# yuriyvnv/speech_transcript_embeddings

Measured on AMD Instinct MI355X. Metric: audio–text pairs/sec (whole node), 10s@16kHz + 64-tok, 1/2/4/8 MI355X, higher is better.
Workload: dtype bf16; 1 GPU; c2: global batch 64 = 1 GPU x 1 micro-batch(es) of 64 pairs, each pair 10s@16kHz audio + 64-tok clean + 64-tok corrupt; w2v-bert-2.0 Conformer 24L + XLM-R-base 12L, 3+3 unfrozen; GPU fbank -> fwd -> InfoNCE -> bwd -> allreduce -> clip+AdamW; global_batch=64, local_batch=64, micro_batch=64, accumulation_steps=1, seq_len_audio_frames=499, seq_len_text=64, parallelism=dp1

## Files before the change

speech_transcript_embeddings_amd/csrc/gemm.hip:

```cpp
#include <atomic>
#include <cstdio>
#include <utility>
#include "common.h"
#include "../../include/ste.h"

namespace {


STE_DEV int km_chunk_xor(int k) { return ((k & 3) | ((k >> 1) & 4)) << 1; }

STE_DEV float apply_act(float v, int act) {
  switch (act) {
    case STE_ACT_SWISH: return swish_f(v);
    case STE_ACT_GELU: return gelu_f(v);
    case STE_ACT_TANH: return tanhf(v);
    case STE_ACT_RELU: return fmaxf(v, 0.0f);
    default: return v;
  }
}
STE_DEV float act_grad(float z, int act) {
  switch (act) {
    case STE_ACT_SWISH_BWD: return swish_d(z);
    case STE_ACT_GELU_BWD: return gelu_d(z);
    case STE_ACT_TANH_BWD_OUT: return 1.0f - z * z;
// ... 449 lines not shown
template <int EF, int ACT, bool FULL>
STE_DEV void epilogue_bf16s(const ste_gemm_args& p, const f32x4 (&acc)[8][4], char* slot, int m0, int n0, int batch,
                            int wm, int wn, int lane_in, const f32x4 (&bias)[4]) {
  static_assert(epi_bf16s<EF>(), "single bf16 output, no operand loads");
  int lane = lane_in;
  asm volatile("" : "+v"(lane));
  constexpr bool FWD = ACT >= STE_ACT_SWISH && ACT <= STE_ACT_RELU;
  const int64_t offC = (int64_t)batch * p.strideC;
  const int c0 = n0 + wn * 32, c1 = n0 + 128 + wn * 32;
  const int rbase = m0 + wm * 128;
  const float alpha = p.alpha;
#pragma unroll
  for (int ps = 0; ps < 4; ++ps) {
    auto value = [&](int ii, int j) {
      f32x4 x = acc[2 * ps + ii][j];
      if constexpr ((EF & EF_BIAS) != 0) x += bias[j];
      x *= alpha;
      if (FWD) x = act4(x, ACT);
      return x;
    };
    bf16s_pass<FULL>(slot, value, (bf16*)p.C + offC, p.ldc, rbase + 2 * ps * 16, p.M, p.N, c0, c1, lane);
  }
}

#ifndef STE_TILE_GROUP
#define STE_TILE_GROUP 8
#endif
STE_HD void tile_of(int t, int num_m, int num_n, int& tm, int& tn) {
  constexpr int GROUP = STE_TILE_GROUP;
  const int group = t / (GROUP * num_n);
  const int first_m = group * GROUP;
  const int gsize = num_m - first_m < GROUP ? num_m - first_m : GROUP;
  tm = first_m + (t % (GROUP * num_n)) % gsize;
  tn = (t % (GROUP * num_n)) / gsize;
}
STE_DEV void map_tile_bid(int bid, int num_m, int num_n, int& batch, int& tm, int& tn) {
  const int tiles = num_m * num_n;
  batch = bid / tiles;
  tile_of(bid - batch * tiles, num_m, num_n, tm, tn);
}
STE_DEV void map_tile(int nwg, int num_m, int num_n, int& batch, int& tm, int& tn) {
  map_tile_bid(xcd_remap(blockIdx.x, nwg), num_m, num_n, batch, tm, tn);
}

namespace small {
constexpr int BM = 128, BN = 128, BK = 64, NT = 256;
constexpr int TILE_BYTES = BM * BK * 2;
constexpr int EPI_BYTES = 4 * 64 * EPI_LD * 4;
constexpr int LDS_BYTES = (4 * TILE_BYTES > EPI_BYTES) ? 4 * TILE_BYTES : EPI_BYTES;

struct Stage {
  bf16x8 v[4];
};

template <bool KC>
STE_DEV void stage_load(Stage& st, const bf16* __restrict__ base, int64_t ld, int row0, int rows, int k0, int K,
                        int tid) {
#pragma unroll
  for (int i = 0; i < 4; ++i) {
    int c = tid + NT * i;
    int r, kk;
    bool ok;
    const bf16* p;
    if (KC) {
      r = c >> 3; kk = (c & 7) * 8;
      ok = (row0 + r < rows) && (k0 + kk < K);
      p = base + (int64_t)(row0 + r) * ld + (k0 + kk);
    } else {
      kk = c >> 4; r = (c & 15) * 8;
      ok = (k0 + kk < K) && (row0 + r < rows);
      p = base + (int64_t)(k0 + kk) * ld + (row0 + r);
    }
    if (ok) st.v[i] = *reinterpret_cast<const bf16x8*>(p);
    else st.v[i] = bf16x8{};
  }
}

template <bool KC>
STE_DEV void stage_store(const Stage& st, char* tile, int tid) {
#pragma unroll
  for (int i = 0; i < 4; ++i) {
    int c = tid + NT * i;
    int off;
    if (KC) {
      int r = c >> 3, ch = c & 7;
      off = r * 128 + ((ch ^ (r & 7)) << 4);
    } else {
      int k = c >> 4, ch = c & 15;
      off = k * 256 + ((ch ^ km_chunk_xor(k)) << 4);
    }
    *reinterpret_cast<bf16x8*>(tile + off) = st.v[i];
  }
}
}

template <bool KC, int KM_ROW_BYTES>
STE_DEV bf16x8 frag_load(const char* tile, int rb, int s, int lane) {
  if (KC) {
    int r = rb + (lane & 15);
    int ch = s * 4 + (lane >> 4);
    return *reinterpret_cast<const bf16x8*>(tile + r * 128 + ((ch ^ (r & 7)) << 4));
  } else {
    int g = lane >> 4, li = lane & 15, q = li >> 2, p = li & 3;
    int k = s * 32 + 8 * g + q;
    int quad = (rb >> 2) + p;
    int a0 = k * KM_ROW_BYTES + ((quad ^ (km_chunk_xor(k) << 1)) << 3);
    int k1 = k + 4;
    int a1 = k1 * KM_ROW_BYTES + ((quad ^ (km_chunk_xor(k1) << 1)) << 3);
    s16x4 lo = ds_read_tr16(tile + a0);
    s16x4 hi = ds_read_tr16(tile + a1);
    return join_tr(lo, hi);
  }
}

template <bool A_KC, bool B_KC>
__global__ __launch_bounds__(small::NT, 2) void gemm_bf16_kernel(ste_gemm_args p) {
  using namespace small;
  extern __shared__ __attribute__((aligned(16))) char smem[];
  const int tid = threadIdx.x, lane = tid & 63, wave = tid >> 6;
  const int wm = wave >> 1, wn = wave & 1;
  const int num_m = (p.M + BM - 1) / BM, num_n = (p.N + BN - 1) / BN;
  int batch, tm, tn;
  map_tile(gridDim.x, num_m, num_n, batch, tm, tn);
  const int m0 = tm * BM, n0 = tn * BN;
  const bf16* A = (const bf16*)p.A + (int64_t)batch * p.strideA;
  const bf16* B = (const bf16*)p.B + (int64_t)batch * p.strideB;

  f32x4 acc[4][4];
#pragma unroll
  for (int i = 0; i < 4; ++i)
#pragma unroll
    for (int j = 0; j < 4; ++j) acc[i][j] = f32x4{0.f, 0.f, 0.f, 0.f};

  const int nk = (p.K + BK - 1) / BK;
  Stage sa, sb;
  stage_load<A_KC>(sa, A, p.lda, m0, p.M, 0, p.K, tid);
  stage_load<B_KC>(sb, B, p.ldb, n0, p.N, 0, p.K, tid);
  stage_store<A_KC>(sa, smem, tid);
  stage_store<B_KC>(sb, smem + TILE_BYTES, tid);
  __syncthreads();

  for (int kt = 0; kt < nk; ++kt) {
    const int cur = kt & 1;
    const bool more = kt + 1 < nk;
    if (more) {
      stage_load<A_KC>(sa, A, p.lda, m0, p.M, (kt + 1) * BK, p.K, tid);
      stage_load<B_KC>(sb, B, p.ldb, n0, p.N, (kt + 1) * BK, p.K, tid);
    }
    const char* ta = smem + cur * 2 * TILE_BYTES;
    const char* tb = ta + TILE_BYTES;
#pragma unroll
    for (int s = 0; s < 2; ++s) {
      bf16x8 fa[4], fb[4];
#pragma unroll
      for (int i = 0; i < 4; ++i) fa[i] = frag_load<A_KC, 256>(ta, wm * 64 + i * 16, s, lane);
#pragma unroll
      for (int j = 0; j < 4; ++j) fb[j] = frag_load<B_KC, 256>(tb, wn * 64 + j * 16, s, lane);
#pragma unroll
      for (int i = 0; i < 4; ++i)
#pragma unroll
        for (int j = 0; j < 4; ++j) acc[i][j] = mfma16(fa[i], fb[j], acc[i][j]);
    }
    if (more) {
      char* na = smem + (cur ^ 1) * 2 * TILE_BYTES;
      stage_store<A_KC>(sa, na, tid);
      stage_store<B_KC>(sb, na + TILE_BYTES, tid);
    }
    __syncthreads();
  }

  float* epi = reinterpret_cast<float*>(smem) + wave * 64 * EPI_LD;
#pragma unroll
  for (int i = 0; i < 4; ++i)
#pragma unroll
    for (int j = 0; j < 4; ++j)
#pragma unroll
      for (int r = 0; r < 4; ++r)
        epi[(i * 16 + (lane >> 4) * 4 + r) * EPI_LD + j * 16 + (lane & 15)] = acc[i][j][r];
  __builtin_amdgcn_s_waitcnt(0xc07f);
  __builtin_amdgcn_wave_barrier();
  Csum csum = {};
  epilogue_tile(p, epi, 64, m0 + wm * 64, n0 + wn * 64, n0 + wn * 64 + 32, batch, lane, csum);
  if (p.colsum)
    colsum_flush(p, csum, n0 + wn * 64, n0 + wn * 64 + 32, batch, lane, ((int64_t)batch * num_m + tm) * 2 + wm);
}

namespace ph8 {
constexpr int NT = 512;
constexpr int HALF = 16384;
constexpr int BUF = 4 * HALF;
constexpr int RING_BYTES = 2 * BUF;
constexpr int EPI_OFF = RING_BYTES;
constexpr int LDS_BYTES = EPI_OFF + 8 * 16 * 64 * 4;

template <int G>
STE_DEV int half_row(int pr, int h) {
  if (G == 128) return h * 128 + pr;
  return (pr / G) * (2 * G) + h * G + (pr % G);
}

template <bool KC, int G, bool O32 = false>
STE_DEV void stage_half(const bf16* base, int64_t ld, int row0, int rows, int k0, int h, char* dst, int wave,
                        int lane) {
#pragma unroll
  for (int i = 0; i < 2; ++i) {
    const int piece = wave * 2 + i;
    const bf16* src;
    if (KC) {
      const int pr = piece * 8 + (lane >> 3);
      const int ch = (lane & 7) ^ (lane >> 3);
      const int gr = min(row0 + half_row<G>(pr, h), rows - 1);
      if (O32) src = (const bf16*)((const char*)base + (uint32_t)(((uint32_t)gr * (uint32_t)ld + k0 + ch * 8) * 2u));
      else src = base + (int64_t)gr * ld + k0 + ch * 8;
    } else {
      const int kk = piece * 4 + (lane >> 4);
      const int lc = (lane & 15) ^ km_chunk_xor(kk);
      const int gc = min(row0 + half_row<G>(lc * 8, h), rows - 8);
      src = base + (int64_t)(k0 + kk) * ld + gc;
    }
    __builtin_amdgcn_global_load_lds((const void*)src, (lds_void*)(dst + piece * 1024), 16, 0, 0);
  }
}
constexpr int SC_OFF = EPI_OFF;
constexpr int SC_STAGE = 2048;
STE_DEV void stage_scales(const Mx8Args& mx, int m0, int M, int n0, int N, int t, char* smem, int wave, int lane) {
  const bool isb = wave >= 4;
  const int r = (wave & 3) * 64 + lane;
  const uint8_t* src = isb ? mx.sb + (uint32_t)(min(n0 + r, N - 1) * (uint32_t)mx.lsb + 4 * t)
                           : mx.sa + (uint32_t)(min(m0 + r, M - 1) * (uint32_t)mx.lsa + 4 * t);
  char* dst = smem + SC_OFF + (t & 1) * SC_STAGE + (isb ? 1024 : 0) + (wave & 3) * 256;
  __builtin_amdgcn_global_load_lds((const void*)src, (lds_void*)dst, 4, 0, 0);
}
template <int OFF>
STE_DEV void ds_u8_lo(int& r, uint32_t addr) {
  asm volatile("ds_read_u8_d16 %0, %1 offset:%2" : "+v"(r) : "v"(addr), "i"(OFF) : "memory");
}
template <int OFF>
STE_DEV void ds_u8_hi(int& r, uint32_t addr) {
  asm volatile("ds_read_u8_d16_hi %0, %1 offset:%2" : "+v"(r) : "v"(addr), "i"(OFF) : "memory");
}
template <int OFF>
STE_DEV void ds_u8(int& r, uint32_t addr) {
  asm volatile("ds_read_u8 %0, %1 offset:%2" : "=v"(r) : "v"(addr), "i"(OFF) : "memory");
}
typedef int i32x8 __attribute__((ext_vector_type(8)));
typedef int i32x4m __attribute__((ext_vector_type(4)));
STE_DEV i32x8 frag_mx(const char* tile, int rb, int lane) {
  const int r = rb + (lane & 15), g = lane >> 4;
  const i32x4m lo = *reinterpret_cast<const i32x4m*>(tile + r * 128 + ((g ^ (r & 7)) << 4));
  const i32x4m hi = *reinterpret_cast<const i32x4m*>(tile + r * 128 + (((g + 4) ^ (r & 7)) << 4));
  return i32x8{lo[0], lo[1], lo[2], lo[3], hi[0], hi[1], hi[2], hi[3]};
}
template <typename F, int... I>
STE_DEV void static_for_impl(F& f, std::integer_sequence<int, I...>) {
  (f(std::integral_constant<int, I>{}), ...);
}
template <int N, typename F>
STE_DEV void static_for(F&& f) {
  static_for_impl(f, std::make_integer_sequence<int, N>{});
}
template <int X, int Y>
STE_DEV f32x4 mfma_mx(const i32x8& x, const i32x8& y, f32x4 c, int sx, int sy) {
  return __builtin_amdgcn_mfma_scale_f32_16x16x128_f8f6f4(x, y, c, 0, 0, 0, sx, 0, sy);
}
}

#define STE_BARRIER() asm volatile("s_barrier" ::: "memory")
#ifdef STE_PRIO_STATIC
#define STE_PRIO_HI()
#define STE_PRIO_LO()
#else
#define STE_PRIO_HI() __builtin_amdgcn_s_setprio(1)
#define STE_PRIO_LO() __builtin_amdgcn_s_setprio(0)
#endif
#define STE_VMCNT(n) asm volatile("s_waitcnt vmcnt(" #n ")" ::: "memory")

STE_DEV bf16x8 frag_load_km_asm(const char* tile, int rb, int s, int lane) {
  const int g = lane >> 4, li = lane & 15, q = li >> 2, pp = li & 3;
  const int k = s * 32 + 8 * g + q;
  const int quad = (rb >> 2) + pp;
  const int k1 = k + 4;
  const s16x4 lo = ds_read_tr16_asm(tile + k * 256 + ((quad ^ (km_chunk_xor(k) << 1)) << 3));
  const s16x4 hi = ds_read_tr16_asm(tile + k1 * 256 + ((quad ^ (km_chunk_xor(k1) << 1)) << 3));
  return join_tr(lo, hi);
}
template <bool B_KC>
STE_DEV bf16x8 frag_b_8ph(const char* tile, int rb, int s, int lane) {
  if (B_KC) return frag_load<true, 256>(tile, rb, s, lane);
  return frag_load_km_asm(tile, rb, s, lane);
}
template <bool A_KC>
STE_DEV bf16x8 frag_a_8ph(const char* tile, int rb, int s, int lane) {
  if (A_KC) return frag_load<true, 256>(tile, rb, s, lane);
  return frag_load_km_asm(tile, rb, s, lane);
}
#define STE_LDS_SYNC(ASM)                               \
  do {                                                  \
    if (ASM) {                                          \
      asm volatile("s_waitcnt lgkmcnt(0)" ::: "memory"); \
      __builtin_amdgcn_sched_barrier(0);                \
    }                                                   \
  } while (0)

STE_DEV f32x8 tile_bias(const ste_gemm_args& p, int n0, int wn, int lane) {
  const int cl = (lane & 7) * 8;
  const int col = cl < 32 ? n0 + wn * 32 + cl : n0 + 128 + wn * 32 + (cl - 32);
  const int nval = p.N - col;
  return nval > 0 ? ld8(p.bias + col, false, nval >= 8, nval) : f32x8{};
}

template <int EF, int ACT, bool FULL>
STE_DEV void epilogue_8ph(const ste_gemm_args& p, const f32x4 (&acc)[8][4], float* epi, int m0, int n0, int batch,
                          int wm, int wn, int lane, f32x8 bias, const Q8Out* q8 = nullptr) {
  Csum csum = {};
  const int c0 = n0 + wn * 32, c1 = n0 + 128 + wn * 32;
#define STE_EPI_STAGE(PS)                                                                       \
  {                                                                                             \
    _Pragma("unroll") for (int j = 0; j < 4; ++j) {                                             \
      _Pragma("unroll") for (int r = 0; r < 4; ++r) {                                           \
        const int row = (lane >> 4) * 4 + r, chunk = (4 * j + ((lane & 15) >> 2)) ^ ((r >> 1) & 1); \
        epi[row * 64 + chunk * 4 + (lane & 3)] = acc[PS][j][r];                                 \
      }                                                                                         \
    }                                                                                           \
    __builtin_amdgcn_s_waitcnt(0xc07f);                                                         \
    __builtin_amdgcn_wave_barrier();                                                            \
  }
#define STE_EPI_ROW0(PS) (m0 + wm * 128 + (PS) * 16)
#define STE_EPI_LOAD(PS, L) epi_load16<EF, ACT, FULL>(p, STE_EPI_ROW0(PS), c0, c1, batch, lane, L);
#define STE_EPI_STORE(PS, L)                                                                    \
  epi_store16<EF, ACT, FULL>(p, epi, STE_EPI_ROW0(PS), c0, c1, batch, lane, bias, L, csum, q8); \
  __builtin_amdgcn_s_waitcnt(0xc07f);                                                           \
  __builtin_amdgcn_wave_barrier();
  if constexpr (EF < 0) {
#define STE_EPI_G(PS)                                                                           \
    STE_EPI_STAGE(PS)                                                                           \
    epilogue_tile(p, epi, 16, STE_EPI_ROW0(PS), c0, c1, batch, lane, csum, 64, true, q8);       \
    __builtin_amdgcn_s_waitcnt(0xc07f);                                                         \
    __builtin_amdgcn_wave_barrier();
    STE_EPI_G(0) STE_EPI_G(1) STE_EPI_G(2) STE_EPI_G(3) STE_EPI_G(4) STE_EPI_G(5) STE_EPI_G(6) STE_EPI_G(7)
#undef STE_EPI_G
  } else {
    EpiLoads L0, L1;
    STE_EPI_LOAD(0, L0)
    STE_EPI_STAGE(0) STE_EPI_LOAD(1, L1) STE_EPI_STORE(0, L0)
    STE_EPI_STAGE(1) STE_EPI_LOAD(2, L0) STE_EPI_STORE(1, L1)
    STE_EPI_STAGE(2) STE_EPI_LOAD(3, L1) STE_EPI_STORE(2, L0)
    STE_EPI_STAGE(3) STE_EPI_LOAD(4, L0) STE_EPI_STORE(3, L1)
    STE_EPI_STAGE(4) STE_EPI_LOAD(5, L1) STE_EPI_STORE(4, L0)
    STE_EPI_STAGE(5) STE_EPI_LOAD(6, L0) STE_EPI_STORE(5, L1)
    STE_EPI_STAGE(6) STE_EPI_LOAD(7, L1) STE_EPI_STORE(6, L0)
    STE_EPI_STAGE(7) STE_EPI_STORE(7, L1)
  }
#undef STE_EPI_STAGE
#undef STE_EPI_ROW0
#undef STE_EPI_LOAD
#undef STE_EPI_STORE
  if (EF < 0 ? p.colsum != nullptr : (EF & EF_COLSUM) != 0)
    colsum_flush(p, csum, c0, c1, batch, lane, ((int64_t)batch * ((p.M + 255) >> 8) + (m0 >> 8)) * 2 + wm);
}

#ifndef STE_EPI_PRE
#define STE_EPI_PRE 1
#endif
template <int EF, int ACT, class Pro>
STE_DEV void epilogue_8ph_pre(const ste_gemm_args& p, const f32x4 (&acc)[8][4], float* epi, int m0, int n0, int batch,
                              int wm, int wn, int lane, f32x8 bias, Pro&& prologue) {
  static_assert(EF >= 0 && (EF & (EF_COLSUM | EF_BETA | EF_RS | EF_Q8)) == 0, "EPI_PRE epilogues");
  Csum csum = {};
  const int c0 = n0 + wn * 32, c1 = n0 + 128 + wn * 32;
#define STE_EPI_STAGE(PS)                                                                       \
  {                                                                                             \
    _Pragma("unroll") for (int j = 0; j < 4; ++j) {                                             \
      _Pragma("unroll") for (int r = 0; r < 4; ++r) {                                           \
        const int row = (lane >> 4) * 4 + r, chunk = (4 * j + ((lane & 15) >> 2)) ^ ((r >> 1) & 1); \
        epi[row * 64 + chunk * 4 + (lane & 3)] = acc[PS][j][r];                                 \
      }                                                                                         \
    }                                                                                           \
    __builtin_amdgcn_s_waitcnt(0xc07f);                                                         \
    __builtin_amdgcn_wave_barrier();                                                            \
  }
#define STE_EPI_ROW0(PS) (m0 + wm * 128 + (PS) * 16)
#define STE_EPI_LOAD(PS, L) epi_load16<EF, ACT, true>(p, STE_EPI_ROW0(PS), c0, c1, batch, lane, L);
#define STE_EPI_STORE(PS, L)                                                                    \
  epi_store16<EF, ACT, true>(p, epi, STE_EPI_ROW0(PS), c0, c1, batch, lane, bias, L, csum);     \
  __builtin_amdgcn_s_waitcnt(0xc07f);                                                           \
  __builtin_amdgcn_wave_barrier();
  EpiLoads L0, L1;
  STE_EPI_LOAD(0, L0) STE_EPI_LOAD(1, L1)
  prologue();
  STE_EPI_STAGE(0) STE_EPI_STORE(0, L0) STE_EPI_LOAD(2, L0)
  STE_EPI_STAGE(1) STE_EPI_STORE(1, L1) STE_EPI_LOAD(3, L1)
  STE_EPI_STAGE(2) STE_EPI_STORE(2, L0) STE_EPI_LOAD(4, L0)
  STE_EPI_STAGE(3) STE_EPI_STORE(3, L1) STE_EPI_LOAD(5, L1)
  STE_EPI_STAGE(4) STE_EPI_STORE(4, L0) STE_EPI_LOAD(6, L0)
  STE_EPI_STAGE(5) STE_EPI_STORE(5, L1) STE_EPI_LOAD(7, L1)
  STE_EPI_STAGE(6) STE_EPI_STORE(6, L0)
  STE_EPI_STAGE(7) STE_EPI_STORE(7, L1)
#undef STE_EPI_STAGE
#undef STE_EPI_ROW0
#undef STE_EPI_LOAD
#undef STE_EPI_STORE
}

template <int W, int E>
STE_DEV void vm_wait8(int extra) {
  constexpr int WE = W + E < 63 ? W + E : 63;
  if (E > 0 && extra) asm volatile("s_waitcnt vmcnt(%0)" ::"n"(WE) : "memory");
  else asm volatile("s_waitcnt vmcnt(%0)" ::"n"(W) : "memory");
}

template <bool A_KC, bool B_KC>
STE_DEV void operand_bases(const ste_gemm_args& p, int batch, const bf16*& A, const bf16*& B, int& nk) {
  if (p.ws_bytes < 0) {
    const int kc = p.K / 64, rem = (int)(-p.ws_bytes - 1);
    const int64_t k0 = ((int64_t)batch * kc + (batch < rem ? batch : rem)) * 64;
    A = (const bf16*)p.A + k0 * (A_KC ? 1 : p.lda);
    B = (const bf16*)p.B + k0 * (B_KC ? 1 : p.ldb);
    nk = kc + (batch < rem ? 1 : 0);
    return;
  }
  A = (const bf16*)p.A + (int64_t)batch * p.strideA;
  B = (const bf16*)p.B + (int64_t)batch * p.strideB;
  nk = p.K / 64;
}

template <bool A_KC, bool B_KC, int EF, int ACT, bool MX = false>
__global__ __launch_bounds__(ph8::NT, 1) void gemm_8ph_kernel(ste_gemm_args p, Mx8Args mx) {
  using namespace ph8;
  constexpr int E_ST = epi_stores<EF>();
  constexpr bool SW = epi_bf16s<EF>();
  constexpr int VW = MX ? 9 : 8;
  static_assert(!MX || (A_KC && B_KC), "MX operands are k-contiguous");
  static_assert(VW <= 63, "vmcnt immediate");
  extern __shared__ __attribute__((aligned(16))) char smem[];
  const int tid = threadIdx.x, lane = tid & 63;
  const int wave = __builtin_amdgcn_readfirstlane(tid >> 6);
  const int wm = wave >> 2, wn = wave & 3;
  const int num_m = (p.M + 255) / 256, num_n = (p.N + 255) / 256;
  const int total = num_m * num_n * p.batch;
  int nk = p.K / 64;
  int vb = blockIdx.x;
  if (vb >= total) return;
  int batch, tm, tn;
  map_tile_bid(xcd_remap(vb, total), num_m, num_n, batch, tm, tn);
  int m0 = tm * 256, n0 = tn * 256;
  const bf16* A;
  const bf16* B;
  operand_bases<A_KC, B_KC>(p, batch, A, B, nk);
#define STAGE_A(t, h) \
  stage_half<A_KC, 64, MX>(A, p.lda, m0, p.M, (t) * 64, h, smem + ((t) & 1) * BUF + (h) * HALF, wave, lane)
#define STAGE_B(t, h) \
  stage_half<B_KC, 128, MX>(B, p.ldb, n0, p.N, (t) * 64, h, smem + ((t) & 1) * BUF + (2 + (h)) * HALF, wave, lane)
#define STAGE_S(t) \
  if constexpr (MX) stage_scales(mx, m0, p.M, n0, p.N, (t), smem, wave, lane)
#define STAGE_PROLOGUE()                                                    \
  {                                                                         \
    STAGE_A(0, 0); STAGE_S(0); STAGE_B(0, 0); STAGE_B(0, 1); STAGE_A(0, 1); \
    if (nk > 1) { STAGE_A(1, 0); STAGE_S(1); STAGE_B(1, 0); }               \
  }
  STAGE_PROLOGUE();
  int extra = 0;
  char* const epi_base = MX ? smem + BUF + (wave < 4 ? HALF : 3 * HALF) + (wave & 3) * EPI16_FLOATS * 4
                            : smem + EPI_OFF + wave * EPI16_FLOATS * 4;
  float* epi = reinterpret_cast<float*>(epi_base);
  constexpr bool EPI_OVL = EF >= 0 && (EF & (EF_Z | EF_R | EF_BETA | EF_COLSUM | EF_RS)) == 0;
  constexpr bool EPI_PRE_OK = EF >= 0 && !EPI_OVL && !MX && !SW && (EF & (EF_Z | EF_R)) != 0 &&
                              (EF & (EF_BETA | EF_COLSUM | EF_RS | EF_Q8 | EF_DROP)) == 0;
  constexpr bool epi_pre = EPI_PRE_OK && STE_EPI_PRE;
  f32x8 bias = f32x8{};
  f32x4 sbias[4] = {};
  if constexpr (EF >= 0 && (EF & EF_BIAS) != 0 && !MX) {
    if constexpr (SW) swap_bias(p, n0, wn, lane, sbias);
    else bias = tile_bias(p, n0, wn, lane);
  }

  for (;;) {
    if (nk > 1) vm_wait8<VW, E_ST>(extra);
    else STE_VMCNT(0);
    STE_BARRIER();

    f32x4 acc[8][4];
#pragma unroll
    for (int i = 0; i < 8; ++i)
#pragma unroll
      for (int j = 0; j < 4; ++j) acc[i][j] = f32x4{0.f, 0.f, 0.f, 0.f};

    bf16x8 a0[4][2], a1[4][2], b0[2][2], b1[2][2];
    i32x8 ma0[MX ? 4 : 1], ma1[MX ? 4 : 1], mb0[MX ? 2 : 1], mb1[MX ? 2 : 1];
    if (wm == 1) STE_BARRIER();
#ifdef STE_PRIO_STATIC
    if (wm == 1) __builtin_amdgcn_s_setprio(1);
#endif
    for (int t = 0; t < nk; ++t) {
      const char* buf = smem + (t & 1) * BUF;
      const bool tail = t + 2 >= nk;
      const int ex = t == 0 ? extra : 0;
      int sca[8] = {0, 0, 0, 0, 0, 0, 0, 0}, scb[4] = {0, 0, 0, 0};
      if constexpr (MX) {
        typedef __attribute__((address_space(3))) char lds_char_t;
        int ln = (int)__builtin_amdgcn_mbcnt_hi(~0u, __builtin_amdgcn_mbcnt_lo(~0u, 0u));
        asm volatile("" : "+v"(ln));
        const uint32_t sbase = (uint32_t)(uintptr_t)(lds_char_t*)smem + SC_OFF + (t & 1) * SC_STAGE + (ln >> 4) +
                               (ln & 15) * 4;
        const uint32_t aa = sbase + wm * 512, ab = sbase + 1024 + wn * 128;
        ds_u8<0>(sca[0], aa);    ds_u8<64>(sca[1], aa);
        ds_u8<128>(sca[2], aa);  ds_u8<192>(sca[3], aa);
        ds_u8<256>(sca[4], aa);  ds_u8<320>(sca[5], aa);
        ds_u8<384>(sca[6], aa);  ds_u8<448>(sca[7], aa);
        ds_u8<0>(scb[0], ab);    ds_u8<64>(scb[1], ab);
        ds_u8<512>(scb[2], ab);  ds_u8<576>(scb[3], ab);
      }
      if constexpr (MX) {
#pragma unroll
        for (int j = 0; j < 2; ++j) mb0[j] = frag_mx(buf + 2 * HALF, wn * 32 + j * 16, lane);
        __builtin_amdgcn_sched_barrier(0);
#pragma unroll
        for (int i = 0; i < 4; ++i) ma0[i] = frag_mx(buf, wm * 64 + i * 16, lane);
      } else {
#pragma unroll
      for (int j = 0; j < 2; ++j)
#pragma unroll
        for (int s = 0; s < 2; ++s) b0[j][s] = frag_b_8ph<B_KC>(buf + 2 * HALF, wn * 32 + j * 16, s, lane);
      __builtin_amdgcn_sched_barrier(0);
#pragma unroll
      for (int i = 0; i < 4; ++i)
#pragma unroll
        for (int s = 0; s < 2; ++s) a0[i][s] = frag_a_8ph<A_KC>(buf, wm * 64 + i * 16, s, lane);
      }
      if (t + 1 < nk) STAGE_B(t + 1, 1);
      if (tail) STE_VMCNT(0); else vm_wait8<VW, E_ST>(ex);
      STE_BARRIER();
      STE_LDS_SYNC(!A_KC || !B_KC || MX);
      STE_PRIO_HI();
      if constexpr (MX) {
        static_for<4>([&](auto ic) {
          constexpr int i = decltype(ic)::value;
          static_for<2>([&](auto jc) {
            constexpr int j = decltype(jc)::value;
            acc[i][j] = SW ? mfma_mx<j, i>(mb0[j], ma0[i], acc[i][j], scb[j], sca[i])
                           : mfma_mx<i, j>(ma0[i], mb0[j], acc[i][j], sca[i], scb[j]);
          });
        });
      } else {
#pragma unroll
      for (int s = 0; s < 2; ++s)
#pragma unroll
        for (int i = 0; i < 4; ++i)
#pragma unroll
          for (int j = 0; j < 2; ++j) acc[i][j] = SW ? mfma16(b0[j][s], a0[i][s], acc[i][j]) : mfma16(a0[i][s], b0[j][s], acc[i][j]);
      }
      STE_PRIO_LO();
      STE_BARRIER();
      if constexpr (MX) {
#pragma unroll
        for (int j = 0; j < 2; ++j) mb1[j] = frag_mx(buf + 3 * HALF, wn * 32 + j * 16, lane);
      } else {
#pragma unroll
      for (int j = 0; j < 2; ++j)
#pragma unroll
        for (int s = 0; s < 2; ++s) b1[j][s] = frag_b_8ph<B_KC>(buf + 3 * HALF, wn * 32 + j * 16, s, lane);
      }
      if (t + 1 < nk) STAGE_A(t + 1, 1);
      if (tail) STE_VMCNT(0); else vm_wait8<VW, E_ST>(ex);
      STE_BARRIER();
      STE_LDS_SYNC(!B_KC);
      STE_PRIO_HI();
      if constexpr (MX) {
        static_for<4>([&](auto ic) {
          constexpr int i = decltype(ic)::value;
          static_for<2>([&](auto jc) {
            constexpr int j = decltype(jc)::value;
            acc[i][2 + j] = SW ? mfma_mx<j, i>(mb1[j], ma0[i], acc[i][2 + j], scb[2 + j], sca[i])
                               : mfma_mx<i, j>(ma0[i], mb1[j], acc[i][2 + j], sca[i], scb[2 + j]);
          });
        });
      } else {
#pragma unroll
      for (int s = 0; s < 2; ++s)
#pragma unroll
        for (int i = 0; i < 4; ++i)
#pragma unroll
          for (int j = 0; j < 2; ++j) acc[i][2 + j] = SW ? mfma16(b1[j][s], a0[i][s], acc[i][2 + j]) : mfma16(a0[i][s], b1[j][s], acc[i][2 + j]);
      }
      STE_PRIO_LO();
      STE_BARRIER();
      if constexpr (MX) {
#pragma unroll
        for (int i = 0; i < 4; ++i) ma1[i] = frag_mx(buf + HALF, wm * 64 + i * 16, lane);
      } else {
#pragma unroll
      for (int i = 0; i < 4; ++i)
#pragma unroll
        for (int s = 0; s < 2; ++s) a1[i][s] = frag_a_8ph<A_KC>(buf + HALF, wm * 64 + i * 16, s, lane);
      }
      if (t + 2 < nk) {
        STAGE_A(t + 2, 0);
        STAGE_S(t + 2);
      }
      STE_BARRIER();
      STE_LDS_SYNC(!A_KC);
      STE_PRIO_HI();
      if constexpr (MX) {
        static_for<4>([&](auto ic) {
          constexpr int i = decltype(ic)::value;
          static_for<2>([&](auto jc) {
            constexpr int j = decltype(jc)::value;
            acc[4 + i][2 + j] = SW ? mfma_mx<j, i>(mb1[j], ma1[i], acc[4 + i][2 + j], scb[2 + j], sca[4 + i])
                                   : mfma_mx<i, j>(ma1[i], mb1[j], acc[4 + i][2 + j], sca[4 + i], scb[2 + j]);
          });
        });
      } else {
#pragma unroll
      for (int s = 0; s < 2; ++s)
#pragma unroll
        for (int i = 0; i < 4; ++i)
#pragma unroll
          for (int j = 0; j < 2; ++j) acc[4 + i][2 + j] = SW ? mfma16(b1[j][s], a1[i][s], acc[4 + i][2 + j]) : mfma16(a1[i][s], b1[j][s], acc[4 + i][2 + j]);
      }
      STE_PRIO_LO();
      STE_BARRIER();
      if (t + 2 < nk) STAGE_B(t + 2, 0);
      if (tail) STE_VMCNT(0); else vm_wait8<VW, E_ST>(ex);
      STE_BARRIER();
      STE_PRIO_HI();
      if constexpr (MX) {
        static_for<4>([&](auto ic) {
          constexpr int i = decltype(ic)::value;
          static_for<2>([&](auto jc) {
            constexpr int j = decltype(jc)::value;
            acc[4 + i][j] = SW ? mfma_mx<j, i>(mb0[j], ma1[i], acc[4 + i][j], scb[j], sca[4 + i])
                               : mfma_mx<i, j>(ma1[i], mb0[j], acc[4 + i][j], sca[4 + i], scb[j]);
          });
        });
      } else {
#pragma unroll
      for (int s = 0; s < 2; ++s)
#pragma unroll
        for (int i = 0; i < 4; ++i)
#pragma unroll
          for (int j = 0; j < 2; ++j) acc[4 + i][j] = SW ? mfma16(b0[j][s], a1[i][s], acc[4 + i][j]) : mfma16(a1[i][s], b0[j][s], acc[4 + i][j]);
      }
      STE_PRIO_LO();
      STE_BARRIER();
    }
    if (wm == 0) STE_BARRIER();

    const int em0 = m0, en0 = n0, ebatch = batch;
    const int vb_next = vb + gridDim.x;
    const bool more = vb_next < total;
    const bool full_tile = em0 + 256 <= p.M && en0 + 256 <= p.N;
    if constexpr (EF >= 0 && (EF & EF_BIAS) != 0 && MX) {
      if constexpr (SW) swap_bias(p, en0, wn, lane, sbias);
      else bias = tile_bias(p, en0, wn, lane);
    } else {
      asm volatile("" : "+v"(bias));
    }
    if constexpr (SW && (EF & EF_BIAS) != 0 && !MX) {
#pragma unroll
      for (int j = 0; j < 4; ++j) asm volatile("" : "+v"(sbias[j]));
    }
    auto next_prologue = [&]() {
      if (more) {
        map_tile_bid(xcd_remap(vb_next, total), num_m, num_n, batch, tm, tn);
        m0 = tm * 256;
        n0 = tn * 256;
        operand_bases<A_KC, B_KC>(p, batch, A, B, nk);
        STAGE_PROLOGUE();
      }
    };
    if (EPI_OVL) next_prologue();
    bool pro_done = EPI_OVL;
    if constexpr (SW) {
      char* slot = epi_base;
      if (full_tile) epilogue_bf16s<EF, ACT, true>(p, acc, slot, em0, en0, ebatch, wm, wn, lane, sbias);
      else epilogue_bf16s<EF, ACT, false>(p, acc, slot, em0, en0, ebatch, wm, wn, lane, sbias);
    } else {
      const Q8Out* q8 = MX && mx.q8.q ? &mx.q8 : nullptr;
      if constexpr (EPI_PRE_OK) {
        if (full_tile && epi_pre) {
          epilogue_8ph_pre<EF, ACT>(p, acc, epi, em0, en0, ebatch, wm, wn, lane, bias, next_prologue);
          pro_done = true;
        } else if (full_tile) {
          epilogue_8ph<EF, ACT, true>(p, acc, epi, em0, en0, ebatch, wm, wn, lane, bias, q8);
        } else {
          epilogue_8ph<EF, ACT, false>(p, acc, epi, em0, en0, ebatch, wm, wn, lane, bias, q8);
        }
      } else {
        if (full_tile) epilogue_8ph<EF, ACT, true>(p, acc, epi, em0, en0, ebatch, wm, wn, lane, bias, q8);
        else epilogue_8ph<EF, ACT, false>(p, acc, epi, em0, en0, ebatch, wm, wn, lane, bias, q8);
      }
    }
    if (!pro_done) next_prologue();
    if (!more) break;
    vb = vb_next;
    extra = ((EPI_OVL || (EPI_PRE_OK && epi_pre)) && full_tile) ? 1 : 0;
    if constexpr (EF >= 0 && (EF & EF_BIAS) != 0 && !MX) {
      if constexpr (SW) swap_bias(p, n0, wn, lane, sbias);
      else bias = tile_bias(p, n0, wn, lane);
    }
  }
#undef STAGE_A
#undef STAGE_B
#undef STAGE_S
#undef STAGE_PROLOGUE
#undef STE_LDS_SYNC
}

int num_cus() {
  static int n = 0;
  if (!n) {
    int dev = 0, v = 0;
    n = (hipGetDevice(&dev) == hipSuccess &&
         hipDeviceGetAttribute(&v, hipDeviceAttributeMultiprocessorCount, dev) == hipSuccess && v > 0) ? v : 256;
  }
  return n;
}

#define STE_EPI_SPECS(X)                                                              \
  X(true, true, EF_BIAS | EF_C2 | EF_CBF16, STE_ACT_SWISH)    \
  X(true, true, EF_BIAS | EF_C2 | EF_CBF16, STE_ACT_GELU)     \
  X(true, true, EF_BIAS | EF_CBF16, STE_ACT_SWISH)            \
  X(true, true, EF_C2 | EF_CBF16, STE_ACT_GELU)               \
  X(true, true, EF_C2, STE_ACT_GELU)                          \
  X(true, true, EF_BIAS | EF_R | EF_DROP, STE_ACT_NONE)       \
  X(true, true, EF_BIAS | EF_C2 | EF_DROP | EF_CBF16, STE_ACT_GELU)  \
  X(true, true, EF_BIAS | EF_CBF16, STE_ACT_GELU)                                     \
  X(true, true, EF_BIAS | EF_C3, STE_ACT_NONE)                \
  X(true, true, EF_BIAS | EF_C2 | EF_C3 | EF_CBF16, STE_ACT_GELU)  \
  X(true, true, EF_BIAS | EF_R, STE_ACT_NONE)                 \
  X(true, true, EF_BIAS | EF_CBF16, STE_ACT_NONE)             \
  X(true, true, EF_CBF16, STE_ACT_NONE)                       \
  X(true, true, EF_R | EF_DROP, STE_ACT_NONE)                 \
  X(true, true, EF_R, STE_ACT_NONE)                                                   \
  X(true, false, EF_CBF16, STE_ACT_NONE)                      \
  X(true, false, 0, STE_ACT_NONE)                             \
  X(true, true, EF_Z | EF_COLSUM | EF_CBF16, STE_ACT_SWISH_BWD)  \
  X(true, true, EF_Z | EF_COLSUM | EF_CBF16, STE_ACT_GELU_BWD)                        \
  X(true, true, EF_Z | EF_COLSUM | EF_C3 | EF_CBF16, STE_ACT_GELU_BWD)  \
  X(true, true, EF_Z | EF_C3 | EF_CBF16, STE_ACT_GELU_BWD)             \
  X(true, true, EF_Z | EF_CBF16, STE_ACT_SWISH_BWD)           \
  X(true, true, EF_Z | EF_CBF16, STE_ACT_GELU_BWD)                                    \
  X(true, true, EF_Z | EF_COLSUM | EF_DROP | EF_CBF16, STE_ACT_GELU_BWD)  \
  X(true, true, EF_Z | EF_DROP | EF_CBF16, STE_ACT_GELU_BWD)  \
  X(true, true, 0, STE_ACT_NONE)                              \
  X(false, false, 0, STE_ACT_NONE)

struct EpiSpec {
  int ef, act;
};
EpiSpec match_epi_spec(bool a_kc, bool b_kc, int ef, int act) {
#define STE_MATCH(AK, BK, E, ACT) \
  if (AK == a_kc && BK == b_kc && ef == (E) && act == (ACT)) return {(E), (ACT)};
  STE_EPI_SPECS(STE_MATCH)
#undef STE_MATCH
  return {EF_GENERIC, 0};
}

template <bool A_KC, bool B_KC>
int launch_8ph(const ste_gemm_args& a, EpiSpec spec, hipStream_t s) {
  const int nb = ((a.M + 255) / 256) * ((a.N + 255) / 256) * a.batch;
  const int grid = nb < num_cus() ? nb : num_cus();
#define STE_TRY(AK, BK, E, ACT)                                                                       \
  if constexpr (AK == A_KC && BK == B_KC) {                                                           \
    if (spec.ef == (E) && spec.act == (ACT)) {                                                        \
      hipLaunchKernelGGL((gemm_8ph_kernel<A_KC, B_KC, (E), (ACT)>), dim3(grid), dim3(ph8::NT),        \
                         ph8::LDS_BYTES, s, a, Mx8Args{});                                            \
      STE_CHECK_LAUNCH();                                                                             \
      return 0;                                                                                       \
    }                                                                                                 \
  }
  STE_EPI_SPECS(STE_TRY)
#undef STE_TRY
  if (spec.ef != EF_GENERIC) return STE_ERR_ARG;
  hipLaunchKernelGGL((gemm_8ph_kernel<A_KC, B_KC, EF_GENERIC, 0>), dim3(grid), dim3(ph8::NT), ph8::LDS_BYTES, s, a,
                     Mx8Args{});
  STE_CHECK_LAUNCH();
  return 0;
}

template <int MAXS>
__global__ __launch_bounds__(256) void splitk_reduce_kernel(float* __restrict__ C, int64_t ldc,
                                                            const float* __restrict__ ws, int M, int N, int S,
                                                            float alpha, float beta) {
  const int n4 = N >> 2;
  const int64_t i = (int64_t)blockIdx.x * blockDim.x + threadIdx.x;
  if (i >= (int64_t)M * n4) return;
  const int64_t slab = (int64_t)M * N;
  const int m = (int)(i / n4), c = (int)(i - (int64_t)m * n4) * 4;
  const float* w = ws + (int64_t)m * N + c;
  float* cp = C + (int64_t)m * ldc + c;
  f32x4 v[MAXS];
#pragma unroll
  for (int k = 0; k < MAXS; ++k) v[k] = *reinterpret_cast<const f32x4*>(w + (k < S ? k : S - 1) * slab);
  const f32x4 cv = beta != 0.f ? *reinterpret_cast<const f32x4*>(cp) : f32x4{0.f, 0.f, 0.f, 0.f};
  f32x4 acc = v[0];
#pragma unroll
  for (int k = 1; k < MAXS; ++k)
    if (k < S) acc += v[k];
  for (int k = MAXS; k < S; ++k) acc += *reinterpret_cast<const f32x4*>(w + k * slab);
  f32x4 out = acc * alpha;
  if (beta != 0.f) out += cv * beta;
  *reinterpret_cast<f32x4*>(cp) = out;
}

__global__ __launch_bounds__(256) void splitk_epi_kernel(ste_gemm_args p, const float* __restrict__ ws, int S) {
  const int n8 = p.N >> 3;
  const int64_t total = (int64_t)p.M * n8;
  const int64_t slab = (int64_t)p.M * p.N;
  const uint32_t thresh = (uint32_t)(p.drop_p * 4294967296.0);
  const float inv_keep = p.drop_p > 0.f ? 1.0f / (1.0f - p.drop_p) : 1.0f;
  Csum csum = {};
  for (int64_t i = (int64_t)blockIdx.x * blockDim.x + threadIdx.x; i < total; i += (int64_t)gridDim.x * blockDim.x) {
    const int row = (int)(i / n8), col = (int)(i - (int64_t)row * n8) * 8;
    const float* w = ws + (int64_t)row * p.N + col;
    f32x4 lo = *reinterpret_cast<const f32x4*>(w), hi = *reinterpret_cast<const f32x4*>(w + 4);
    for (int k = 1; k < S; ++k) {
      lo += *reinterpret_cast<const f32x4*>(w + k * slab);
      hi += *reinterpret_cast<const f32x4*>(w + k * slab + 4);
    }
    const f32x8 bias = p.bias ? ld8(p.bias + col, false, true, 8) : f32x8{};
    epi_apply8(p, f32x8{lo[0], lo[1], lo[2], lo[3], hi[0], hi[1], hi[2], hi[3]}, row, col, true, 8, bias, thresh,
               inv_keep, 0, 0, csum, nullptr, 0);
  }
}

template <bool A_KC, bool B_KC>
int launch_small(const ste_gemm_args& a, hipStream_t s) {
  using namespace small;
  const int num_m = (a.M + BM - 1) / BM, num_n = (a.N + BN - 1) / BN;
  const int nb = num_m * num_n * a.batch;
  hipLaunchKernelGGL((gemm_bf16_kernel<A_KC, B_KC>), dim3(nb), dim3(NT), LDS_BYTES, s, a);
  STE_CHECK_LAUNCH();
  return 0;
}

bool env_is(const char* e, char c) { return e && e[0] == c; }

bool small_only() {
  static const bool on = env_is(STE_AB_ENV("STE_GEMM_SMALL_ONLY"), '1');
  return on;
}

std::atomic<int> g_min_tiles_bf16{-1}, g_min_tiles_mx8{240};
int min_tiles_bf16() {
  int v = g_min_tiles_bf16.load();
  if (v < 0) {
    const char* e = STE_AB_ENV("STE_GEMM_MIN_TILES");
    const int dflt = e ? atoi(e) : 240;
    if (g_min_tiles_bf16.compare_exchange_strong(v, dflt)) v = dflt;
  }
  return v;
}

int tiles_256(const ste_gemm_args& a) { return ((a.M + 255) / 256) * ((a.N + 255) / 256); }

bool ph8_shape_ok(const ste_gemm_args& a) {
  if (a.K % 64) return false;
  if (!a.a_kc || a.M < 8) return false;
  if (!a.b_kc && (a.N % 8)) return false;
  return true;
}

bool plain_epilogue(const ste_gemm_args& a) {
  return !(a.bias || a.C2 || a.C3 || a.R || a.Z || a.colsum || a.row_scale || a.act || a.drop_p > 0.f);
}

int few_split_slabs(const ste_gemm_args& a) {
  static const bool off = env_is(STE_AB_ENV("STE_GEMM_FEW_SPLIT"), '0');
  if (off || !a.a_kc || !a.b_kc || !a.ws || a.batch != 1 || a.colsum || !ph8_shape_ok(a)) return 0;
  if ((a.N & 7) || a.K / 64 < 40 || a.M < 2048) return 0;
  if (tiles_256(a) * 2 > num_cus()) return 0;
  if (2 * (int64_t)a.M * a.N * 4 > a.ws_bytes) return 0;
  return 2;
}

bool batched_dw_ok(const ste_gemm_args& a) {
  static const bool off = env_is(STE_AB_ENV("STE_GEMM_BATCHED_DW"), '0');
  if (off || a.a_kc || a.b_kc || a.batch < 2 || !plain_epilogue(a)) return false;
  if ((a.M & 7) || (a.N & 7) || a.M < 256 || a.N < 256 || a.K < 1024) return false;
  return (long)tiles_256(a) * a.batch >= 240;
}

int dw_split_slabs(const ste_gemm_args& a) {
  if (a.a_kc || a.b_kc || !a.ws || a.batch != 1 || !plain_epilogue(a) || a.c_bf16) return 0;
  if ((a.M & 7) || (a.N & 7)) return 0;
  const int nk = a.K / 64, tiles = tiles_256(a);
  if (nk < 16 || tiles > 256) return 0;
  int S = 256 / tiles;
  if (S > nk / 8) S = nk / 8;
  const int64_t slab = (int64_t)a.M * a.N * 4;
  while (S > 1 && S * slab > a.ws_bytes) --S;
  return (S < 1 || S * slab > a.ws_bytes) ? 0 : S;
}

enum class GemmPath { Small, Ph8, DwSplitK, BatchedDw, FewSplit };
struct GemmPlan {
  GemmPath path;
  int variant;
  int S, Kc, rem;
  int64_t k8;
  int64_t cs_rows;
  EpiSpec spec;
};

GemmPlan plan_gemm(const ste_gemm_args& a) {
  GemmPlan pl = {};
  pl.path = GemmPath::Small;
  pl.variant = (a.a_kc ? 0 : 2) + (a.b_kc ? 0 : 1);
  pl.spec = {EF_GENERIC, 0};
  const int nk = a.K / 64;
  const int min_tiles = min_tiles_bf16();
  if (!small_only()) {
    if ((pl.S = dw_split_slabs(a)) > 0) pl.path = GemmPath::DwSplitK;
    else if (batched_dw_ok(a)) pl.path = GemmPath::BatchedDw;
    else if ((pl.S = few_split_slabs(a)) > 0) pl.path = GemmPath::FewSplit;
    else if (ph8_shape_ok(a) && (long)tiles_256(a) * a.batch >= min_tiles) pl.path = GemmPath::Ph8;
  }
  switch (pl.path) {
    case GemmPath::DwSplitK:
    case GemmPath::FewSplit:
      pl.Kc = nk / pl.S;
      pl.rem = nk - pl.S * pl.Kc;
      pl.k8 = (int64_t)nk * 64;
      pl.spec = match_epi_spec(a.a_kc, a.b_kc, 0, STE_ACT_NONE);
      break;
    case GemmPath::BatchedDw:
      pl.k8 = (int64_t)nk * 64;
      pl.spec = match_epi_spec(false, false, epi_flags(a), a.act);
      break;
    case GemmPath::Ph8:
      pl.spec = match_epi_spec(true, a.b_kc, epi_flags(a), a.act);
      [[fallthrough]];
    case GemmPath::Small:
      if (a.colsum) {
        const int bm = pl.path == GemmPath::Ph8 ? 256 : small::BM;
        const int64_t rows = 2 * (int64_t)((a.M + bm - 1) / bm);
        if (a.ws && a.ws_bytes >= rows * a.batch * a.N * 4) pl.cs_rows = rows;
      }
      break;
  }
  return pl;
}

ste_gemm_args slab_args(const ste_gemm_args& a, const GemmPlan& pl) {
  ste_gemm_args g = a;
  g.K = pl.Kc * 64;
  g.batch = pl.S;
  g.ws = nullptr;
  g.ws_bytes = -(int64_t)(pl.rem + 1);
  g.bias = nullptr; g.C2 = nullptr; g.C3 = nullptr; g.R = nullptr; g.Z = nullptr; g.colsum = nullptr;
  g.row_scale = nullptr; g.act = 0; g.drop_p = 0.f;
  g.C = a.ws; g.ldc = a.N; g.strideC = (int64_t)a.M * a.N; g.c_bf16 = 0;
  g.alpha = 1.f; g.beta = 0.f;
  return g;
}

int launch_k_tail(const ste_gemm_args& a, int64_t kdone, hipStream_t s) {
  ste_gemm_args r = a;
  r.K = (int)(a.K - kdone);
  r.A = (const bf16*)a.A + kdone * a.lda;
  r.B = (const bf16*)a.B + kdone * a.ldb;
  r.beta = 1.f;
  r.ws = nullptr;
  return launch_small<false, false>(r, s);
}

int check_gemm_args(const ste_gemm_args& a) {
  if (a.M <= 0 || a.N <= 0 || a.K <= 0) return STE_ERR_ARG;
  auto misaligned = [&a](const void* ptr, int64_t ld, int esz) {
    return a.N >= 8 && ptr && ((((uintptr_t)ptr) & 15) || ((ld * esz) & 15));
  };
  if (misaligned(a.C, a.ldc, a.c_bf16 ? 2 : 4) || misaligned(a.C2, a.ldc2, 2) || misaligned(a.C3, a.ldc3, 2) ||
      misaligned(a.R, a.ldr, a.r_bf16 ? 2 : 4) || misaligned(a.Z, a.ldz, 2) || misaligned(a.bias, 0, 4))
    return STE_ERR_SHAPE;
  return 0;
}

}

extern "C" int ste_gemm_kernel(const ste_gemm_args* args) {
  if (!args) return STE_ERR_ARG;
  ste_gemm_args a = *args;
  if (a.batch <= 0) a.batch = 1;
  const GemmPlan pl = plan_gemm(a);
  switch (pl.path) {
    case GemmPath::Small: return STE_GEMM_KERNEL_SMALL + pl.variant;
    case GemmPath::Ph8:
    case GemmPath::BatchedDw: return STE_GEMM_KERNEL_8PH + pl.variant;
    case GemmPath::DwSplitK:
    case GemmPath::FewSplit: return STE_GEMM_KERNEL_SPLITK + pl.variant;
  }
  return STE_ERR_ARG;
}

extern "C" int ste_gemm_kernel_name(const ste_gemm_args* args, char* buf, int len) {
  if (!args || !buf || len <= 0) return STE_ERR_ARG;
  ste_gemm_args a = *args;
  if (a.batch <= 0) a.batch = 1;
  const GemmPlan pl = plan_gemm(a);
  const char* ak = (pl.variant & 2) ? "false" : "true";
  const char* bk = (pl.variant & 1) ? "false" : "true";
  if (pl.path == GemmPath::Small) snprintf(buf, len, "gemm_bf16_kernel<%s, %s>", ak, bk);
  else snprintf(buf, len, "gemm_8ph_kernel<%s, %s, %d, %d>", ak, bk, pl.spec.ef, pl.spec.act);
  return 0;
}

extern "C" int ste_gemm(const ste_gemm_args* args, void* stream) {
// ... 312 lines not shown
```

Before: 500.6 pairs/s.

## Pipeline transposed LDS fragment reads with counted lgkmcnt waits in GEMM main loop

For GEMM variants with K-major (transposed) operands, the main loop now issues LDS fragment reads in s-halves. It replaces the full lgkmcnt(0) wait before each MFMA block with counted waits, so the first MFMAs can start while later ds_read_b64_tr_b16 loads are still in flight. It also precomputes per-lane swizzled LDS base addresses once and uses immediate offsets, flipping the base between double buffers each iteration, which cuts per-read address arithmetic. The risk is that wrong wait counts cause races, and the extra address registers add pressure.

```diff
diff --git a/speech_transcript_embeddings_amd/csrc/gemm.hip b/speech_transcript_embeddings_amd/csrc/gemm.hip
--- a/speech_transcript_embeddings_amd/csrc/gemm.hip
+++ b/speech_transcript_embeddings_amd/csrc/gemm.hip
@@ -775,6 +775,27 @@
     }                                                   \
   } while (0)
 
+#ifndef STE_KM_PIPE
+#define STE_KM_PIPE 1
+#endif
+#ifndef STE_KM_IMM
+#define STE_KM_IMM 1
+#endif
+template <int OFF>
+STE_DEV bf16x8 frag_km_imm(uint32_t base) {
+  static_assert(OFF >= 0 && OFF + 1024 < 65536, "ds offset field");
+  s16x4 lo, hi;
+  asm volatile("ds_read_b64_tr_b16 %0, %1 offset:%2" : "=v"(lo) : "v"(base), "n"(OFF) : "memory");
+  asm volatile("ds_read_b64_tr_b16 %0, %1 offset:%2" : "=v"(hi) : "v"(base), "n"(OFF + 1024) : "memory");
+  return join_tr(lo, hi);
+}
+template <int N>
+STE_DEV void lds_wait_counted() {
+  __builtin_amdgcn_sched_barrier(0);
+  asm volatile("s_waitcnt lgkmcnt(%0)" ::"n"(N < 15 ? N : 15) : "memory");
+  __builtin_amdgcn_sched_barrier(0);
+}
+
 STE_DEV f32x8 tile_bias(const ste_gemm_args& p, int n0, int wn, int lane) {
   const int cl = (lane & 7) * 8;
   const int col = cl < 32 ? n0 + wn * 32 + cl : n0 + 128 + wn * 32 + (cl - 32);
@@ -931,6 +952,20 @@
     STAGE_A(0, 0); STAGE_S(0); STAGE_B(0, 0); STAGE_B(0, 1); STAGE_A(0, 1); \
     if (nk > 1) { STAGE_A(1, 0); STAGE_S(1); STAGE_B(1, 0); }               \
   }
+  constexpr int PIPE = (MX || (A_KC && B_KC)) ? 0 : STE_KM_PIPE;
+  static_assert(PIPE == 0 || PIPE == 1, "STE_KM_PIPE");
+  constexpr int RA = A_KC ? 0 : 2, RB = B_KC ? 0 : 2;
+  constexpr bool IMM = STE_KM_IMM && PIPE == 1;
+#define RD_A(dst, h, i, s, b)                                                                       \
+  if constexpr (IMM && !A_KC) dst[i][s] = frag_km_imm<(h) * HALF + (s) * 8192>(abase[i]);           \
+  else dst[i][s] = frag_a_8ph<A_KC>((b) + (h) * HALF, wm * 64 + (i) * 16, s, lane)
+#define RD_B(dst, h, j, s)                                                                          \
+  if constexpr (IMM && !B_KC) dst[j][s] = frag_km_imm<(2 + (h)) * HALF + (s) * 8192>(bbase[j]);     \
+  else dst[j][s] = frag_b_8ph<B_KC>(buf + (2 + (h)) * HALF, wn * 32 + (j) * 16, s, lane)
+#define MM(I0, J0, AF, BF, s, ILO, IHI)                                                                \
+  _Pragma("unroll") for (int i = ILO; i < IHI; ++i) _Pragma("unroll") for (int j = 0; j < 2; ++j)      \
+    acc[(I0) + i][(J0) + j] = SW ? mfma16(BF[j][s], AF[i][s], acc[(I0) + i][(J0) + j])                 \
+                                 : mfma16(AF[i][s], BF[j][s], acc[(I0) + i][(J0) + j])
   STAGE_PROLOGUE();
   int extra = 0;
   char* const epi_base = MX ? smem + BUF + (wave < 4 ? HALF : 3 * HALF) + (wave & 3) * EPI16_FLOATS * 4
@@ -964,6 +999,27 @@
 #ifdef STE_PRIO_STATIC
     if (wm == 1) __builtin_amdgcn_s_setprio(1);
 #endif
+    uint32_t abase[4] = {}, bbase[2] = {};
+    if constexpr (IMM) {
+      typedef __attribute__((address_space(3))) char lds_char_t;
+      const int kq = 8 * (lane >> 4) + ((lane & 15) >> 2), pp = lane & 3;
+      const int X = km_chunk_xor(kq) << 1;
+      const uint32_t row = (uint32_t)(uintptr_t)(lds_char_t*)smem + kq * 256;
+      if constexpr (!A_KC) {
+#pragma unroll
+        for (int i = 0; i < 4; ++i) {
+          abase[i] = row + (((((wm * 64 + i * 16) >> 2) + pp) ^ X) << 3);
+          asm volatile("" : "+v"(abase[i]));
+        }
+      }
+      if constexpr (!B_KC) {
+#pragma unroll
+        for (int j = 0; j < 2; ++j) {
+          bbase[j] = row + (((((wn * 32 + j * 16) >> 2) + pp) ^ X) << 3);
+          asm volatile("" : "+v"(bbase[j]));
+        }
+      }
+    }
     for (int t = 0; t < nk; ++t) {
       const char* buf = smem + (t & 1) * BUF;
       const bool tail = t + 2 >= nk;
@@ -989,6 +1045,16 @@
         __builtin_amdgcn_sched_barrier(0);
 #pragma unroll
         for (int i = 0; i < 4; ++i) ma0[i] = frag_mx(buf, wm * 64 + i * 16, lane);
+      } else if constexpr (PIPE == 1) {
+        RD_B(b0, 0, 0, 0); RD_B(b0, 0, 1, 0);
+        __builtin_amdgcn_sched_barrier(0);
+#pragma unroll
+        for (int i = 0; i < 4; ++i) RD_A(a0, 0, i, 0, buf);
+        __builtin_amdgcn_sched_barrier(0);
+        RD_B(b0, 0, 0, 1); RD_B(b0, 0, 1, 1);
+        __builtin_amdgcn_sched_barrier(0);
+#pragma unroll
+        for (int i = 0; i < 4; ++i) RD_A(a0, 0, i, 1, buf);
       } else {
 #pragma unroll
       for (int j = 0; j < 2; ++j)
@@ -1003,7 +1069,8 @@
       if (t + 1 < nk) STAGE_B(t + 1, 1);
       if (tail) STE_VMCNT(0); else vm_wait8<VW, E_ST>(ex);
       STE_BARRIER();
-      STE_LDS_SYNC(!A_KC || !B_KC || MX);
+      STE_LDS_SYNC((!A_KC || !B_KC || MX) && PIPE == 0);
+      if constexpr (PIPE == 1) lds_wait_counted<2 * RA + 2 * RB + 4 * RA>();
       STE_PRIO_HI();
       if constexpr (MX) {
         static_for<4>([&](auto ic) {
@@ -1014,6 +1081,14 @@
                            : mfma_mx<i, j>(ma0[i], mb0[j], acc[i][j], sca[i], scb[j]);
           });
         });
+      } else if constexpr (PIPE == 1) {
+        MM(0, 0, a0, b0, 0, 0, 2);
+        lds_wait_counted<2 * RB + 4 * RA>();
+        MM(0, 0, a0, b0, 0, 2, 4);
+        lds_wait_counted<2 * RA>();
+        MM(0, 0, a0, b0, 1, 0, 2);
+        lds_wait_counted<0>();
+        MM(0, 0, a0, b0, 1, 2, 4);
       } else {
 #pragma unroll
       for (int s = 0; s < 2; ++s)
@@ -1027,6 +1102,10 @@
       if constexpr (MX) {
 #pragma unroll
         for (int j = 0; j < 2; ++j) mb1[j] = frag_mx(buf + 3 * HALF, wn * 32 + j * 16, lane);
+      } else if constexpr (PIPE >= 1) {
+        RD_B(b1, 1, 0, 0); RD_B(b1, 1, 1, 0);
+        __builtin_amdgcn_sched_barrier(0);
+        RD_B(b1, 1, 0, 1); RD_B(b1, 1, 1, 1);
       } else {
 #pragma unroll
       for (int j = 0; j < 2; ++j)
@@ -1036,7 +1115,8 @@
       if (t + 1 < nk) STAGE_A(t + 1, 1);
       if (tail) STE_VMCNT(0); else vm_wait8<VW, E_ST>(ex);
       STE_BARRIER();
-      STE_LDS_SYNC(!B_KC);
+      STE_LDS_SYNC(!B_KC && PIPE == 0);
+      if constexpr (PIPE >= 1) lds_wait_counted<2 * RB>();
       STE_PRIO_HI();
       if constexpr (MX) {
         static_for<4>([&](auto ic) {
@@ -1047,6 +1127,10 @@
                                : mfma_mx<i, j>(ma0[i], mb1[j], acc[i][2 + j], sca[i], scb[2 + j]);
           });
         });
+      } else if constexpr (PIPE >= 1) {
+        MM(0, 2, a0, b1, 0, 0, 4);
+        lds_wait_counted<0>();
+        MM(0, 2, a0, b1, 1, 0, 4);
       } else {
 #pragma unroll
       for (int s = 0; s < 2; ++s)
@@ -1060,6 +1144,12 @@
       if constexpr (MX) {
 #pragma unroll
         for (int i = 0; i < 4; ++i) ma1[i] = frag_mx(buf + HALF, wm * 64 + i * 16, lane);
+      } else if constexpr (PIPE >= 1) {
+#pragma unroll
+        for (int i = 0; i < 4; ++i) RD_A(a1, 1, i, 0, buf);
+        __builtin_amdgcn_sched_barrier(0);
+#pragma unroll
+        for (int i = 0; i < 4; ++i) RD_A(a1, 1, i, 1, buf);
       } else {
 #pragma unroll
       for (int i = 0; i < 4; ++i)
@@ -1071,7 +1161,8 @@
         STAGE_S(t + 2);
       }
       STE_BARRIER();
-      STE_LDS_SYNC(!A_KC);
+      STE_LDS_SYNC(!A_KC && PIPE == 0);
+      if constexpr (PIPE >= 1) lds_wait_counted<2 * RA + 4 * RA>();
       STE_PRIO_HI();
       if constexpr (MX) {
         static_for<4>([&](auto ic) {
@@ -1082,6 +1173,14 @@
                                    : mfma_mx<i, j>(ma1[i], mb1[j], acc[4 + i][2 + j], sca[4 + i], scb[2 + j]);
           });
         });
+      } else if constexpr (PIPE >= 1) {
+        MM(4, 2, a1, b1, 0, 0, 2);
+        lds_wait_counted<4 * RA>();
+        MM(4, 2, a1, b1, 0, 2, 4);
+        lds_wait_counted<2 * RA>();
+        MM(4, 2, a1, b1, 1, 0, 2);
+        lds_wait_counted<0>();
+        MM(4, 2, a1, b1, 1, 2, 4);
       } else {
 #pragma unroll
       for (int s = 0; s < 2; ++s)
@@ -1115,6 +1214,13 @@
       }
       STE_PRIO_LO();
       STE_BARRIER();
+      if constexpr (IMM) {
+        const int d = (t & 1) ? -BUF : BUF;
+#pragma unroll
+        for (int i = 0; i < 4; ++i) abase[i] += A_KC ? 0 : d;
+#pragma unroll
+        for (int j = 0; j < 2; ++j) bbase[j] += B_KC ? 0 : d;
+      }
     }
     if (wm == 0) STE_BARRIER();
 
@@ -1176,6 +1282,9 @@
 #undef STAGE_B
 #undef STAGE_S
 #undef STAGE_PROLOGUE
+#undef RD_A
+#undef RD_B
+#undef MM
 #undef STE_LDS_SYNC
 }
 
```

Result: no change. 503.2 pairs/s (median of 6 runs) (+0.5%).
